# GuildOfWeavers/genSTARK

Measured on AMD Instinct MI355X. Metric: prove() ms + NTT GF(p) elements/sec, MiMC-128 2^20 steps, higher is better.
Workload: dtype u128; 1 GPU; MiMC-128 prove(), 2^20 steps, extensionFactor 16, exeQueryCount 48, friQueryCount 64, blake2s256; one independent proof per GPU; evaluation_domain=16777216, ntt_points_per_prove=17827072, ntt_transforms_per_prove=4, proof_bytes=371695

## Files before the change

### genstark_amd/_abi.py

```python
import ctypes as C
import os

_HERE = os.path.dirname(os.path.abspath(__file__))
HIP_LIB_PATH = os.path.join(_HERE, 'csrc', 'libgstark_hip.so')
MODULUS_128 = 2**128 - 9 * 2**32 + 1
MODULUS_64 = 2**64 - 21 * 2**30 + 1
MODULUS_32 = 2**32 - 3 * 2**25 + 1
MODULUS_17 = 96769
MODULUS_256 = 2**256 - 351 * 2**32 + 1
MODULUS_224 = 2**224 - 2**96 + 1
HIP_LIB_PATHS = {MODULUS_128: HIP_LIB_PATH, MODULUS_64: os.path.join(_HERE, 'csrc', 'libgstark_hip_q64.so'),
                 MODULUS_32: os.path.join(_HERE, 'csrc', 'libgstark_hip_q32.so'),
                 MODULUS_17: os.path.join(_HERE, 'csrc', 'libgstark_hip_q17.so'),
                 MODULUS_256: os.path.join(_HERE, 'csrc', 'libgstark_hip_p256.so'),
                 MODULUS_224: os.path.join(_HERE, 'csrc', 'libgstark_hip_p224.so')}
HIP_LIB_PATH_RUNTIME = os.path.join(_HERE, 'csrc', 'libgstark_hip_rt.so')

GS_OK = 0


class FriLayer(C.Structure):
    _fields_ = [('next', C.c_void_p), ('leaves', C.c_void_p), ('nodes', C.c_void_p), ('point_out', C.c_void_p), ('ticket', C.c_uint64)]

HASH_ALGS = {'sha256': 0, 'blake2s256': 1}
# ... 99 lines not shown
OPTIONAL_SYMBOLS = tuple(_OPTIONAL_SIGNATURES)

_HADES_SIGNATURES = {
    'gs_hades_create': (_int, [_vp, _u32, _u32, _u32, _u64, _bytes, _bytes, _pvp]),
    'gs_hades_destroy': (_int, [_vp, _vp]),
    'gs_hades_hash': (_int, [_vp, _vp, _vp, _u64, _u32, _u32, _vp]),
    'gs_hades_merkle': (_int, [_vp, _vp, _vp, _u64, _u32, _vp]),
    'gs_hades_merkle_paths': (_int, [_vp, _vp, _u64, _u32, C.POINTER(_u64), _u64, _vp]),
    'gs_hades_merkle_top': (_u32, []),
}
HADES_SYMBOLS = tuple(_HADES_SIGNATURES)

_RESCUE_SIGNATURES = {
    'gs_rescue_create': (_int, [_vp, _u32, _u32, _u64, _bytes, _bytes, _bytes, _pvp]),
    'gs_rescue_destroy': (_int, [_vp, _vp]),
    'gs_rescue_hash': (_int, [_vp, _vp, _vp, _u64, _u32, _u32, _u32, _u32, _vp]),
    'gs_rescue_merkle': (_int, [_vp, _vp, _vp, _u64, _vp]),
    'gs_rescue_spread_limit': (_u64, []),
}
RESCUE_SYMBOLS = tuple(_RESCUE_SIGNATURES)

_TREE_UPDATE_SIGNATURES = {
    'gs_hades_merkle_update': (_int, [_vp, _vp, _vp, _u64, _u32, C.POINTER(_u64), _vp, _u64, _vp, _vp]),
    'gs_rescue_merkle_update': (_int, [_vp, _vp, _vp, _u64, C.POINTER(_u64), _vp, _u64, _vp, _vp]),
}
TREE_UPDATE_SYMBOLS = tuple(_TREE_UPDATE_SIGNATURES)

_TREE_VERIFY_SIGNATURES = {
    'gs_hades_merkle_path_roots': (_int, [_vp, _vp, _vp, _u32, _u32, C.POINTER(_u64), _vp, _u64, _vp]),
    'gs_rescue_merkle_path_roots': (_int, [_vp, _vp, _vp, _u32, C.POINTER(_u64), _vp, _u64, _vp]),
}
TREE_VERIFY_SYMBOLS = tuple(_TREE_VERIFY_SIGNATURES)


class GstarkError(RuntimeError):
    pass


def load_library(path):
    if not os.path.exists(path):
        raise GstarkError(
            f'{path} not found: the HIP backend is not built (run `python -c "import __graft_entry__ as g; g.build()"`).'
            ' There is no CPU fallback.')
    lib = C.CDLL(path)
    for name, (res, args) in _SIGNATURES.items():
        fn = getattr(lib, name)
        fn.restype, fn.argtypes = res, args
    for name, (res, args) in (list(_OPTIONAL_SIGNATURES.items()) + list(_HADES_SIGNATURES.items()) + list(_RESCUE_SIGNATURES.items())
                              + list(_TREE_UPDATE_SIGNATURES.items()) + list(_TREE_VERIFY_SIGNATURES.items())):
        fn = getattr(lib, name, None)
        if fn is not None:
            fn.restype, fn.argtypes = res, args
    return lib


class Backend:

    def __init__(self, device=0, stream=None, lib_path=None, allow_test_double=False, modulus=None):
        if lib_path is None:
            lib_path = HIP_LIB_PATH if modulus is None else HIP_LIB_PATHS.get(modulus, HIP_LIB_PATH_RUNTIME)
        self.lib = load_library(lib_path)
        self.element_size = self.lib.gs_element_size()
        if modulus is not None:
            if modulus < 3 or modulus >> (8 * self.element_size):
                raise GstarkError(f'a modulus of {modulus.bit_length()} bits does not fit {lib_path}')
            rc = self.lib.gs_set_modulus(modulus.to_bytes(self.element_size, 'little'), self.element_size)
            if rc != GS_OK:
                raise GstarkError(f'{lib_path} does not compute modulo {modulus} (gs_set_modulus: {rc}'
                                  + (': the runtime-modulus library serves ONE modulus per process, and it has been given another' if rc == -3 else '') + ')')
        buf = C.create_string_buffer(self.element_size)
        self.lib.gs_field_modulus(C.cast(buf, C.c_void_p))
        self.modulus = int.from_bytes(buf.raw, 'little')
        if modulus is not None and self.modulus != modulus:
            raise GstarkError(f'{lib_path} is built for the field of {self.modulus} elements, not {modulus}')
        if not self.modulus:
            raise GstarkError(f'{lib_path} takes its modulus at run time: pass modulus=')
        self.name = self.lib.gs_backend_name().decode()
        if self.name != 'hip-gfx950' and not allow_test_double:
            raise GstarkError(f'refusing backend {self.name!r}: the product path runs on hip-gfx950 only')
        if self.lib.gs_abi_version() != 1:
            raise GstarkError('gstark ABI version mismatch')
        ctx = C.c_void_p()
# ... 86 lines not shown
```

### genstark_amd/csrc/air_mimc.hip

```cpp
#include "common.h"
#include "host_field.h"

__global__ void k_mimc_constraints(const fe *__restrict__ p, uint64_t nc, uint64_t shift, const fe *__restrict__ k, uint64_t klen,
                                   fe *__restrict__ out) {
    for (uint64_t j = blockIdx.x * (uint64_t)blockDim.x + threadIdx.x; j < nc; j += (uint64_t)gridDim.x * blockDim.x) {
        uint64_t jn = j + shift;
        if (jn >= nc) jn -= nc;
        fe x = p[j], nx = p[jn];
        fe x3 = fe_mul(fe_mul(x, x), x);
        out[j] = fe_sub(nx, fe_add(x3, k[j % klen]));
    }
}

#define GS_MIMC_COMP_MAX_PERIOD 32
#define GS_MIMC_COMP_MAX_ROOTS 4
struct MimcCompArgs {
    fe qz[GS_MIMC_COMP_MAX_PERIOD];
    fe bt[GS_MIMC_COMP_MAX_PERIOD];
    fe lt[GS_MIMC_COMP_MAX_PERIOD];
    fe ipoly[GS_MIMC_COMP_MAX_ROOTS];
    uint64_t root[GS_MIMC_COMP_MAX_ROOTS];
    fe x_last;
};
__global__ void k_mimc_composition(const fe *__restrict__ p, uint64_t n, uint64_t shift, const fe *__restrict__ k, uint64_t klen,
                                   const fe *__restrict__ tw_lo, const fe *__restrict__ tw_hi, int log_lo, int logn, const fe *__restrict__ u,
                                   MimcCompArgs a, uint32_t period, uint32_t nroots, int with_lc, fe *__restrict__ out) {
    __shared__ fe qz[GS_MIMC_COMP_MAX_PERIOD], bt[GS_MIMC_COMP_MAX_PERIOD], lt[GS_MIMC_COMP_MAX_PERIOD];
    if (threadIdx.x < period) { qz[threadIdx.x] = a.qz[threadIdx.x]; bt[threadIdx.x] = a.bt[threadIdx.x]; lt[threadIdx.x] = a.lt[threadIdx.x]; }
    __syncthreads();
    for (uint64_t i = blockIdx.x * (uint64_t)blockDim.x + threadIdx.x; i < n; i += (uint64_t)gridDim.x * blockDim.x) {
        fe x = tw_lo[i & ((1ull << log_lo) - 1)];
        if (logn > log_lo) x = fe_mul(x, tw_hi[i >> log_lo]);
        const fe pi = p[i], pn = p[(i + shift) & (n - 1)];
        const fe q = fe_sub(pn, fe_add(fe_mul(fe_mul(pi, pi), pi), k[i % klen]));
        const fe d = fe_mul(fe_mul(q, fe_sub(x, a.x_last)), qz[i & (period - 1)]);
        fe iv = a.ipoly[nroots - 1];
        for (int c = (int)nroots - 2; c >= 0; c--) iv = fe_add(fe_mul(iv, x), a.ipoly[c]);
        fe b = fe_mul(fe_sub(pi, iv), bt[i & (period - 1)]);
        for (uint32_t r = 0; r < nroots; r++) b = fe_mul(b, u[(i + n - a.root[r]) & (n - 1)]);
        fe r = fe_add(d, b);
        if (with_lc) r = fe_add(r, fe_mul(pi, lt[i & (period - 1)]));
        out[i] = r;
    }
}

#define GS_MIMC_CHUNK_BODY(STEP)                                                                                \
    for (uint64_t i = base; i < end; i++) {                                                                    \
        t[i] = hf_mimc_out(x);                                      \
        x = STEP(x, rc[ri]);                                   \
        if (++ri == nrc) ri = 0;                                                                               \
    }                                                                                                          \
    *ri_io = ri;                                                                                               \
    return x;
static hfe mimc_chunk_generic(hfe *t, hfe x, const hfe *rc, uint32_t nrc, uint32_t *ri_io, uint64_t base, uint64_t end) {
    uint32_t ri = *ri_io;
    GS_MIMC_CHUNK_BODY(hf_mimc_step_weak)
}
#if defined(__x86_64__) && !defined(__HIP_DEVICE_COMPILE__) && defined(GS_FIELD_128)
#define GS_MIMC_CHUNK_V3 1
__attribute__((target("arch=x86-64-v3,tune=znver5"))) static hfe mimc_chunk_v3(hfe *t, hfe x, const hfe *rc, uint32_t nrc, uint32_t *ri_io, uint64_t base,
                                                                               uint64_t end) {
    uint32_t ri = *ri_io;
    GS_MIMC_CHUNK_BODY(hf_cube_add_rows)
}
#endif
extern "C" {

int gs_mimc_trace(gs_ctx *c, const gs_elt *seed, const uint8_t *rc_host, uint32_t nrc, uint64_t steps, void *out) {
    if (!c || !seed || !rc_host || !out) return GS_ERR_ARG;
    if (!nrc || !steps) return gs_fail(c, GS_ERR_ARG, "mimc_trace: empty");
    std::vector<hfe> rc(nrc);
    for (uint32_t i = 0; i < nrc; i++) rc[i] = hf_load(rc_host + GS_ELT * i);
    int rcode = gs_trace_begin(c, steps * GS_ELT);
    if (rcode) return rcode;
    hfe *t = (hfe *)c->h_trace;
    hfe x = hf_load(seed);
    uint32_t ri = 0;
    const uint64_t CHUNK = 1ull << 16;
#ifdef GS_MIMC_CHUNK_V3
    static const bool v3 = __builtin_cpu_supports("avx2") && __builtin_cpu_supports("bmi2") && __builtin_cpu_supports("fma");
#else
    const bool v3 = false;
#endif
    for (uint64_t base = 0; base < steps; base += CHUNK) {
        const uint64_t end = base + CHUNK < steps ? base + CHUNK : steps;
#ifdef GS_MIMC_CHUNK_V3
        if (v3) x = mimc_chunk_v3(t, x, rc.data(), nrc, &ri, base, end);
        else
#endif
            x = mimc_chunk_generic(t, x, rc.data(), nrc, &ri, base, end);
        (void)v3;
        GS_HIP(c, hipMemcpyAsync((uint8_t *)out + base * GS_ELT, t + base, (end - base) * GS_ELT, hipMemcpyHostToDevice, c->stream));
    }
    return gs_trace_end(c);
}

int gs_mimc_constraints(gs_ctx *c, const void *p_comp, uint64_t nc, uint64_t shift, const void *k_table, uint64_t klen, void *out) {
    if (!c || !p_comp || !k_table || !out) return GS_ERR_ARG;
    if (!nc || !klen) return gs_fail(c, GS_ERR_ARG, "mimc_constraints: empty");
    hipLaunchKernelGGL(k_mimc_constraints, dim3(gs_grid(nc)), dim3(256), 0, c->stream, (const fe *)p_comp, nc, shift % nc,
                       (const fe *)k_table, klen, (fe *)out);
    GS_LAUNCH_CHECK(c);
    return GS_OK;
}

int gs_mimc_composition(gs_ctx *c, const void *p_eval, uint64_t n, uint64_t steps, const gs_elt *omega, const void *k_table, uint64_t klen,
                        const uint8_t *coeffs_host, uint64_t q_inc, uint64_t b_inc, const uint8_t *ipoly_host, const uint64_t *root_index_host,
                        uint32_t nroots, const uint8_t *lc_coeffs_host, void *out) {
    if (!c || !p_eval || !omega || !k_table || !coeffs_host || !ipoly_host || !root_index_host || !out) return GS_ERR_ARG;
    if (!gs_is_pow2(n) || !gs_is_pow2(steps) || steps > n || !klen) return gs_fail(c, GS_ERR_ARG, "mimc_composition: bad sizes");
    const uint64_t period = n / steps;
    if (period > GS_MIMC_COMP_MAX_PERIOD || nroots == 0 || nroots > GS_MIMC_COMP_MAX_ROOTS)
        return gs_fail(c, GS_ERR_UNSUPPORTED, "mimc_composition: n / steps <= %d and 1..%d assertions", GS_MIMC_COMP_MAX_PERIOD, GS_MIMC_COMP_MAX_ROOTS);
    if (q_inc % steps || b_inc % steps) return gs_fail(c, GS_ERR_ARG, "mimc_composition: degree increments must be multiples of the trace length");
    const fe w = fe_from_bytes(omega);
    const fe *lo, *hi, *u;
    int log_lo;
    int rc = gs_plan_pow_tables(c, w, n, &lo, &hi, &log_lo);
    if (!rc) rc = gs_plan_inverse_table(c, w, n, &u);
    if (rc) return rc;
    const fe d0 = fe_from_bytes(coeffs_host), d1 = fe_from_bytes(coeffs_host + GS_ELT), b0 = fe_from_bytes(coeffs_host + 2 * GS_ELT),
             b1 = fe_from_bytes(coeffs_host + 3 * GS_ELT);
    const fe l0 = lc_coeffs_host ? fe_from_bytes(lc_coeffs_host) : fe_zero(), l1 = lc_coeffs_host ? fe_from_bytes(lc_coeffs_host + GS_ELT) : fe_zero();
    MimcCompArgs a;
    uint64_t ksum = 0;
    for (uint32_t r = 0; r < GS_MIMC_COMP_MAX_ROOTS; r++) {
        a.root[r] = r < nroots ? root_index_host[r] & (n - 1) : 0;
        a.ipoly[r] = r < nroots ? fe_from_bytes(ipoly_host + GS_ELT * r) : fe_zero();
        if (r < nroots) ksum = (ksum + a.root[r]) & (n - 1);
    }
    const fe scale = gs_memo_pow(c, w, (n - ksum) & (n - 1));
    const std::vector<fe> &tab = gs_memo(c, gs_memo_key("mimc_comp").add(w).add(n).add(steps).add(q_inc).add(b_inc), [&](std::vector<fe> &t) {
        const fe g = fe_pow_u64(w, steps);
        const fe gq = fe_pow_u64(g, (q_inc / steps) % period), gb = fe_pow_u64(g, (b_inc / steps) % period);
        fe gj = fe_one(), gqj = fe_one(), gbj = fe_one();
        for (uint64_t j = 0; j < period; j++) {
            t.push_back(fe_inv(fe_sub(gj, fe_one())));
            t.push_back(gqj);
            t.push_back(gbj);
            gj = fe_mul(gj, g); gqj = fe_mul(gqj, gq); gbj = fe_mul(gbj, gb);
        }
        t.push_back(fe_pow_u64(w, (steps - 1) * period));
    });
    for (uint64_t j = 0; j < GS_MIMC_COMP_MAX_PERIOD; j++) {
        if (j < period) {
            a.qz[j] = fe_mul(fe_add(d0, fe_mul(d1, tab[3 * j + 1])), tab[3 * j]);
            a.bt[j] = fe_mul(fe_add(b0, fe_mul(b1, tab[3 * j + 2])), scale);
            a.lt[j] = fe_add(l0, fe_mul(l1, tab[3 * j + 2]));
        } else {
            a.qz[j] = a.bt[j] = a.lt[j] = fe_zero();
        }
    }
    a.x_last = tab[3 * period];
    gs_traffic(c, 2 * n * GS_ELT, n, "k_mimc_composition");
    hipLaunchKernelGGL(k_mimc_composition, dim3(gs_grid(n)), dim3(256), 0, c->stream, (const fe *)p_eval, n, period, (const fe *)k_table, klen, lo, hi,
                       log_lo, gs_log2(n), u, a, (uint32_t)period, nroots, lc_coeffs_host ? 1 : 0, (fe *)out);
    GS_LAUNCH_CHECK(c);
    return GS_OK;
}

}
```

### genstark_amd/csrc/common.h

```cpp
#pragma once
#include <hip/hip_runtime.h>
#include <stdint.h>
#include <stdio.h>
#include <stdarg.h>
#include <string.h>

#include <array>

#include <map>
#include <mutex>
#include <string>
#include <vector>

#include "../../include/gstark.h"
#if defined(GS_SMALL_Q)
#include "gf_small.h"
#elif defined(GS_WIDE_BITS)
#include "gf_wide.h"
#else
#include "gf128.h"
#define GS_FIELD_128 1
#endif

#if defined(GF_RUNTIME_MODULUS)
// ... 7 lines not shown

#define GS_ELT ((uint64_t)sizeof(fe))
#define GS_EW ((uint32_t)(sizeof(fe) / 16))
#ifndef GF_LIMBS
#define GF_LIMBS 4
GF_HD uint32_t fe_limb(const fe &a, int i) { return i == 0 ? a.w0 : (i == 1 ? a.w1 : (i == 2 ? a.w2 : a.w3)); }
GF_HD void fe_set_limb(fe &a, int i, uint32_t v) { if (i == 0) a.w0 = v; else if (i == 1) a.w1 = v; else if (i == 2) a.w2 = v; else a.w3 = v; }
#else
GF_HD uint32_t fe_limb(const fe &a, int i) { return a.w[i]; }
GF_HD void fe_set_limb(fe &a, int i, uint32_t v) { a.w[i] = v; }
#endif

struct NttPlan;

#define GS_HOST_TRACE_MAX_SEGMENTS 8

struct gs_ctx {
    int device = 0;
    hipStream_t stream = nullptr;
    bool own_stream = false;
    char err[512] = {0};
    std::mutex blocks_mutex;
    std::multimap<uint64_t, void *> free_blocks;
    std::map<void *, uint64_t> live_blocks;
    uint64_t cached_bytes = 0;
    std::map<std::string, NttPlan *> plans;
    void *h_stage = nullptr;
    void *h_stage_dev = nullptr;
    void *d_stage = nullptr;
    uint64_t stage_bytes = 0;
    void *fri_x = nullptr;
    void *fri_points = nullptr;
    std::map<std::string, std::vector<fe>> scalar_memo;
    uint64_t jit_launches = 0;
    bool traffic_on = false;
    std::map<std::string, std::array<uint64_t, 3>> traffic;
    uint64_t host_trace_segments = GS_HOST_TRACE_MAX_SEGMENTS;
    int air_jit = 2;
    struct DeferredCopy { void *dst; uint64_t first_word, bytes; };
    bool defer = false;
    std::vector<uint64_t> defer_addrs;
    std::vector<DeferredCopy> defer_copies;
    void *h_trace = nullptr;
    uint64_t trace_bytes = 0;
    hipEvent_t trace_done = nullptr;
    bool trace_pending = false;
    static constexpr uint32_t RB_SLOTS = 64, RB_SLOT_BYTES = 256;
    void *h_rb = nullptr, *h_rb_dev = nullptr;
    uint32_t rb_bytes[RB_SLOTS] = {};
    uint64_t rb_next = 0;
    void *h_fl = nullptr, *h_fl_dev = nullptr, *d_fl_count = nullptr;
    uint64_t fl_bytes = 0, fl_seq = 0;
    static constexpr uint64_t UP_HALF = 8ull << 20;
    void *h_up = nullptr;
    uint64_t up_off = 0;
    int up_half = 0;
    hipEvent_t up_done[2] = {};
    bool up_pending[2] = {false, false};
};

int gs_fail(gs_ctx *c, int code, const char *fmt, ...);

static inline void gs_traffic(gs_ctx *c, uint64_t bytes, uint64_t units, const char *fmt, ...) __attribute__((format(printf, 4, 5)));
static inline void gs_traffic(gs_ctx *c, uint64_t bytes, uint64_t units, const char *fmt, ...) {
    if (!c->traffic_on) return;
    char name[64];
// ... 74 lines not shown
```

### genstark_amd/csrc/gf128.h

```cpp
#pragma once
#include <stdint.h>

#if defined(__HIPCC__)
#define GF_HD __host__ __device__ __forceinline__
#else
#define GF_HD inline
#endif

struct alignas(16) fe {
    uint32_t w0, w1, w2, w3;
};

#define GF_P0 0x00000001u
#define GF_P1 0xFFFFFFF7u
#define GF_P2 0xFFFFFFFFu
#define GF_P3 0xFFFFFFFFu

GF_HD fe fe_make(uint32_t a, uint32_t b, uint32_t c, uint32_t d) { fe r; r.w0 = a; r.w1 = b; r.w2 = c; r.w3 = d; return r; }
GF_HD fe fe_zero() { return fe_make(0, 0, 0, 0); }
GF_HD fe fe_one() { return fe_make(1, 0, 0, 0); }
GF_HD bool fe_is_zero(const fe &a) { return (a.w0 | a.w1 | a.w2 | a.w3) == 0; }
GF_HD bool fe_eq(const fe &a, const fe &b) { return a.w0 == b.w0 && a.w1 == b.w1 && a.w2 == b.w2 && a.w3 == b.w3; }

GF_HD bool fe_ge_p(const fe &a) {
// ... 75 lines not shown
    o[2] = (uint32_t)t;
    t = (uint64_t)ai * b[3] + (t >> 32);
    o[3] = (uint32_t)t;
    o[4] = (uint32_t)(t >> 32);
}

GF_HD void fe_mul_wide(const fe &a, const fe &b, uint32_t r[8]) {
    const uint32_t bv[4] = {b.w0, b.w1, b.w2, b.w3};
    uint32_t r0[5], r1[5], r2[5], r3[5], c;
    fe_row_mul(a.w0, bv, r0);
    fe_row_mul(a.w1, bv, r1);
    fe_row_mul(a.w2, bv, r2);
    fe_row_mul(a.w3, bv, r3);
    r[0] = r0[0];
    r[1] = gf_addc(r0[1], r1[0], 0u, c);
    r[2] = gf_addc(r0[2], r1[1], c, c);
    r[3] = gf_addc(r0[3], r1[2], c, c);
    r[4] = gf_addc(r0[4], r1[3], c, c);
    r[5] = r1[4] + c;
    r[2] = gf_addc(r[2], r2[0], 0u, c);
    r[3] = gf_addc(r[3], r2[1], c, c);
    r[4] = gf_addc(r[4], r2[2], c, c);
    r[5] = gf_addc(r[5], r2[3], c, c);
    r[6] = r2[4] + c;
    r[3] = gf_addc(r[3], r3[0], 0u, c);
    r[4] = gf_addc(r[4], r3[1], c, c);
    r[5] = gf_addc(r[5], r3[2], c, c);
    r[6] = gf_addc(r[6], r3[3], c, c);
    r[7] = r3[4] + c;
}

GF_HD uint32_t gf_fsh(uint32_t hi, uint32_t lo, int s) { return (hi << s) | (lo >> (32 - s)); }

GF_HD fe fe_reduce_wide(const uint32_t r[8]) {
    uint32_t c, b;
    uint64_t m = (uint64_t)r[4] * 9u;
    uint32_t a0 = (uint32_t)m;
    m = (uint64_t)r[5] * 9u + (m >> 32);
    uint32_t a1 = (uint32_t)m;
    m = (uint64_t)r[6] * 9u + (m >> 32);
    uint32_t a2 = (uint32_t)m;
    m = (uint64_t)r[7] * 9u + (m >> 32);
    uint32_t a3 = (uint32_t)m, a4 = (uint32_t)(m >> 32);
    uint32_t u1 = gf_addc(r[1], a0, 0u, c);
    uint32_t u2 = gf_addc(r[2], a1, c, c);
    uint32_t u3 = gf_addc(r[3], a2, c, c);
    uint32_t u4 = gf_addc(a3, 0u, c, c);
    uint32_t u5 = a4 + c;
    uint32_t v0 = gf_subc(r[0], r[4], 0u, b);
    uint32_t v1 = gf_subc(u1, r[5], b, b);
    uint32_t v2 = gf_subc(u2, r[6], b, b);
    uint32_t v3 = gf_subc(u3, r[7], b, b);
    uint32_t t0 = gf_subc(u4, 0u, b, b);
    uint32_t t1 = u5 - b;
    uint32_t g0 = gf_addc(t0 << 3, t0, 0u, c);
    uint32_t g1 = gf_fsh(t1, t0, 3) + t1 + c;
    uint32_t e0 = gf_subc(0u, t0, 0u, b);
    uint32_t e1 = gf_subc(g0, t1, b, b);
    uint32_t e2 = g1 - b;
    fe w;
    uint32_t k;
    w.w0 = gf_addc(v0, e0, 0u, c);
    w.w1 = gf_addc(v1, e1, c, c);
    w.w2 = gf_addc(v2, e2, c, c);
    w.w3 = gf_addc(v3, 0u, c, k);
    fe t;
    t.w0 = gf_addc(w.w0, 0xFFFFFFFFu, 0u, c);
    t.w1 = gf_addc(w.w1, 8u, c, c);
    t.w2 = gf_addc(w.w2, 0u, c, c);
    t.w3 = gf_addc(w.w3, 0u, c, c);
    bool sel = (k | c) != 0;
    fe o;
    o.w0 = sel ? t.w0 : w.w0;
    o.w1 = sel ? t.w1 : w.w1;
    o.w2 = sel ? t.w2 : w.w2;
    o.w3 = sel ? t.w3 : w.w3;
    return o;
}

GF_HD fe fe_mul(const fe &a, const fe &b) {
    uint32_t r[8];
    fe_mul_wide(a, b, r);
    return fe_reduce_wide(r);
}
GF_HD fe fe_sqr(const fe &a) { return fe_mul(a, a); }

GF_HD fe fe_pow(fe b, const fe &e) {
    fe r = fe_one();
    const uint32_t ev[4] = {e.w0, e.w1, e.w2, e.w3};
    for (int i = 0; i < 4; i++) {
        uint32_t w = ev[i];
        for (int k = 0; k < 32; k++) {
            if (w & 1u) r = fe_mul(r, b);
            b = fe_sqr(b);
            w >>= 1;
        }
    }
    return r;
}
GF_HD fe fe_pow_u64(fe b, uint64_t e) {
    if (!e) return fe_one();
    fe r = b;
    bool have = false;
    for (;;) {
        if (e & 1u) { r = have ? fe_mul(r, b) : b; have = true; }
        e >>= 1;
        if (!e) break;
        b = fe_sqr(b);
    }
    return r;
// ... 35 lines not shown
```

### genstark_amd/csrc/prover.cc

```cpp
#include <dlfcn.h>
#include <stdarg.h>
#include <stdio.h>

#include <algorithm>
#include <map>
#include <chrono>
#include <deque>
#include <string>
#include <vector>

#include "../../include/gstark.h"
#include "../../include/gstark_prover.h"
#include "../../include/gstark_comm.h"
#include "../../include/gstark_boundary.h"
#if defined(GS_WIDE_BITS)
#include "gf_wide.h"
#endif
#include "host_field.h"
#include "host_poly.h"
#include "host_hash.h"

namespace {

#define GS_API_LIST(X)                                                                                                        \
    X(gs_alloc) X(gs_free) X(gs_upload) X(gs_download) X(gs_gather) X(gs_last_error) X(gs_power_series) X(gs_vec_add) X(gs_vec_mul) \
    X(gs_vec_sub_scalar) X(gs_vec_div) X(gs_combine_many) X(gs_combine_adjusted) X(gs_pluck) X(gs_transpose_vector) X(gs_sub_matrix_from_vectors)     \
    X(gs_eval_polys_at_roots) X(gs_interpolate_roots) X(gs_interpolate_quartic_domain) X(gs_eval_quartic_batch)                \
    X(gs_hash_merge_rows) X(gs_hash_digest_values) X(gs_merkle_build) X(gs_merkle_commit_rows) X(gs_merkle_prove_batch) X(gs_small_interpolate)          \
    X(gs_small_eval_poly) X(gs_pseudorandom_indexes) X(gs_mimc_trace) X(gs_mimc_constraints) X(gs_air_trace)                    \
    X(gs_air_trace_segments) X(gs_air_constraints) X(gs_air_constraints_strided) X(gs_composition_tail) X(gs_composition_tail_coset) X(gs_zero_poly_inverses) X(gs_div_by_domain_roots) X(gs_mimc_composition) X(gs_fri_fold) X(gs_fri_fold_seeded) X(gs_defer_begin) X(gs_defer_end) X(gs_readback_post) X(gs_readback_wait) X(gs_merkle_commit_rows_seed) X(gs_fri_fold_at) \
    X(gs_vec_mul_scalar) X(gs_copy) X(gs_gather_words) X(gs_transpose_records) X(gs_fri_fold_seeded_scaled) X(gs_fri_layers) X(gs_sync) X(gs_zero_poly_inverses_coset) X(gs_div_by_domain_roots_coset)
#define GS_API_OPTIONAL_LIST(X) X(gs_boundary_polys) X(gs_eval_polys_at_points)
struct Api {
#define X(name) decltype(&::name) name = nullptr;
    GS_API_LIST(X)
    GS_API_OPTIONAL_LIST(X)
#undef X
};
Api g_default_api;
bool g_bound = false;
thread_local const Api *g_api = &g_default_api;
#define A (*g_api)
struct UseApi {
    const Api *saved;
    explicit UseApi(const Api *a) : saved(g_api) { g_api = a; }
    ~UseApi() { g_api = saved; }
};

struct Fail {
    int code;
    std::string msg;
};
[[noreturn]] void fail(int code, const char *fmt, ...) {
    char buf[512];
    va_list ap;
    va_start(ap, fmt);
    vsnprintf(buf, sizeof buf, fmt, ap);
    va_end(ap);
    throw Fail{code, buf};
}

typedef hfe F;
const uint64_t ELEM = HF_ELT;
const uint64_t DIGEST = 32, MAX_ARRAY = 256;
const uint64_t WORD = 16, EW = ELEM / WORD;
// ... 900 lines not shown
    Plan plan = make_plan(job, T, E, omega, false);
    const uint64_t Nc = plan.Nc, combination_degree = plan.combination_degree, b_inc = plan.b_inc;
    const F comp_rou = hf_pow(omega, (hfe)(N / Nc)), exec_rou = hf_pow(omega, (hfe)E);
    const Coset domain{N, omega, 1, E, true};


    uint32_t assertions_on_r0 = 0;
    for (uint32_t i = 0; i < job.nassertions; i++) assertions_on_r0 += job.assertions[i].reg == 0;
    const bool fused = air.kind == 0 && E <= 32 && air.nconstraints == 1 && assertions_on_r0 == job.nassertions && job.nassertions <= 4;
    const bool tail = !fused && tail_fits(job, R + air.nsecret);
    const bool tail_makes_z = tail && domain.unit <= 32;
    uint32_t most_assertions = 0;
    for (auto &r : plan.regs) most_assertions = std::max(most_assertions, (uint32_t)r.steps.size());
    const uint32_t DEVICE_BOUNDARY_ABOVE = 128;
    const bool device_boundary = !fused && !tail && most_assertions > DEVICE_BOUNDARY_ABOVE && A.gs_boundary_polys && !g_host_boundary && plan.regs.size() <= 64 &&
                                 most_assertions <= T && T <= (1ull << 28);
    if (!device_boundary) plan.fill_xs();
    Buf zInverses;
    if (!fused && !tail_makes_z) zInverses = zero_poly_inverses(x, plan, domain);
    Buf psbPowers;
    const bool lc_folds = fused && R + air.nsecret == 1;
    if (b_inc > 0 && !lc_folds && !tail) psbPowers = coset_powers(x, domain, b_inc);

    Buf kN;
    uint64_t klen_n = 0;
    if (air.kind == 0) {
        klen_n = air.k_len * (N / Nc);
        Buf kPoly(x, air.k_len * ELEM);
        kN = Buf(x, klen_n * ELEM);
        x.check(counted_interpolate_roots(x.c, air.k_table, 1, enc(hf_pow(omega, (hfe)(N / air.k_len))), air.k_len, kPoly.p), "gs_interpolate_roots(K)");
        x.check(counted_eval_polys_at_roots(x.c, kPoly.p, 1, air.k_len, enc(hf_pow(omega, (hfe)(N / klen_n))), klen_n, kN.p), "gs_eval_polys_at_roots(K)");
    }

    clock.mark("context + trace-independent work issued");
    clock.readme(x, "Set up evaluation context");
    Buf trace(x, (uint64_t)R * T * ELEM);
    launch_trace(x, job, air.first_rows, air.segments, trace.p);
    check_assertion_ranges(job);
    std::vector<uint64_t> asserted_at;
    for (uint32_t i = 0; i < job.nassertions; i++) asserted_at.push_back((uint64_t)job.assertions[i].reg * T + job.assertions[i].step);

    clock.mark("execution trace (host recurrence)");
    clock.readme(x, "Generated execution trace");
    Buf pPolys(x, (uint64_t)R * T * ELEM), pEval(x, (uint64_t)R * N * ELEM);
    x.check(counted_interpolate_roots(x.c, trace.p, R, enc(exec_rou), T, pPolys.p), "gs_interpolate_roots(trace)");
    clock.readme(x, "Computed execution trace polynomials P(x)");
    x.check(counted_eval_polys_at_roots(x.c, pPolys.p, R, T, enc(omega), N, pEval.p), "gs_eval_polys_at_roots(P)");
    clock.readme(x, "Low-degree extended P(x) polynomials over evaluation domain");
    std::vector<const void *> pRows(R);
    for (uint32_t r = 0; r < R; r++) pRows[r] = pEval.at((uint64_t)r * N * ELEM);
    std::vector<const void *> eVectors(pRows);
    for (uint32_t i = 0; i < air.nsecret; i++) eVectors.push_back(air.secret_traces[i]);
    const uint32_t V = (uint32_t)eVectors.size();

    Tree eTree = commit_rows(x, alg, eVectors.data(), V, N, false);

    clock.mark("P(x), extension, evaluation tree issued");
    clock.readme(x, "Serialized evaluations of P(x) and S(x) polynomials + Built evaluation merkle tree (one fused call)");
    const uint32_t dcount = plan.dcount, bcoef = plan.bcoef;
    std::vector<F> coefficients;
    auto read_evaluation_root = [&] {
        Bytes got(asserted_at.size() * ELEM);
        const uint64_t one = 1;
        DeferWindow win(x);
        x.check(A.gs_gather(x.c, trace.p, ELEM, asserted_at.data(), asserted_at.size(), got.data()), "gs_gather(asserted cells)");
        x.check(A.gs_gather(x.c, eTree.nodes.p, DIGEST, &one, 1, eTree.root.data()), "gs_gather(root)");
        win.end();
        check_asserted_cells(job, [&](uint32_t i) { return got.data() + i * ELEM; });
        trace.release();
        coefficients = plan.coefficients(eTree.root, V);
    };

    Buf cEval(x, N * ELEM);
    bool lc_fused = false;
    if (fused) {
        const Plan::Boundary bd = plan.boundary(E, true);
        read_evaluation_root();
        const bool q_adjusted = plan.groups[0].first < combination_degree;
        Bytes co(4 * ELEM, 0);
        store_elem(coefficients[0], co.data());
        if (q_adjusted) store_elem(coefficients[1], co.data() + ELEM);
        store_elem(coefficients[dcount], co.data() + 2 * ELEM);
        if (b_inc > 0) store_elem(coefficients[dcount + 1], co.data() + 3 * ELEM);
        lc_fused = lc_folds;
        Bytes lc = lc_folds ? pack(coefficients, dcount + bcoef, plan.lccount(V)) : Bytes();
        lc.resize(2 * ELEM, 0);
        x.check(A.gs_mimc_composition(x.c, pRows[0], N, T, enc(omega), kN.p, klen_n, co.data(), q_adjusted ? combination_degree - plan.groups[0].first : 0, b_inc,
                                      bd.interpolants.data(), bd.at.data(), bd.per_row[0], lc_folds ? lc.data() : nullptr, cEval.p), "gs_mimc_composition");
    } else {
        const bool direct = air.kind == 0;
        const Coset qDomain = direct ? domain : Coset{Nc, comp_rou, 1, Nc / T, true};
        const uint64_t Nq = qDomain.n;
        Buf q(x, (uint64_t)air.nconstraints * Nq * ELEM);
        if (direct) {
            x.check(A.gs_mimc_constraints(x.c, pRows[0], N, N / T, kN.p, klen_n, q.p), "gs_mimc_constraints");
        } else {
            x.check(A.gs_air_constraints_strided(x.c, air.e_code, air.e_ninstr, air.consts, air.nconsts, air.vm_regs, R, air.nconstraints, pEval.p, N, N / Nc,
                                                 Nc, Nc / T, air.static_tables, air.static_lens, air.nstatic, q.p), "gs_air_constraints_strided");
        }
        std::vector<const void *> qa;
        for (uint32_t i = 0; i < air.nconstraints; i++) qa.push_back(q.at((uint64_t)i * Nq * ELEM));
        read_evaluation_root();
        Buf qe(x, N * ELEM), qc;
        if (!direct) qc = Buf(x, Nc * ELEM);
        merge_q(x, plan, coefficients, qa, Nq, [&](uint64_t e) { return coset_powers(x, qDomain, e); }, direct ? qe.p : qc.p);
        if (!direct) {
            Buf qcPoly(x, Nc * ELEM);
            x.check(counted_interpolate_roots(x.c, qc.p, 1, enc(comp_rou), Nc, qcPoly.p), "gs_interpolate_roots(Q)");
            x.check(counted_eval_polys_at_roots(x.c, qcPoly.p, 1, Nc, enc(omega), N, qe.p), "gs_eval_polys_at_roots(Q)");
        }
        std::vector<const void *> pv;
        for (auto &r : plan.regs) pv.push_back(pRows[r.reg]);
        if (tail) {
            composition_tail(x, plan, domain, coefficients, qe.p, tail_makes_z ? nullptr : zInverses.p, pv, eVectors, cEval.p);
            lc_fused = true;
        } else {
            member_sequence(x, plan, domain, device_boundary, coefficients, qe, zInverses, pv, psbPowers, cEval.p);
        }
    }
    zInverses.release();

// ... 92 lines not shown
```

Before: 1.667 billion elements/s.

## Precompute cached X/U/IU tables for MiMC composition and fuse the reduction dot product

Adds a prepare step, issued before trace generation, that builds three device tables. They hold x - x_last, the product of shifted inverse values for the assertion roots, and that product multiplied by the boundary interpolant. X and U are cached in the context by domain and root keys; IU is rebuilt whenever the interpolant changes. The composition kernel then reads these tables instead of evaluating powers, gathering inverse entries and running the interpolant Horner loop per point. It also combines the three final products with a single lazy 128-bit reduction (new fe_reduce_wide9). The cost is three extra N-element buffers, a large amount of memory at this domain size, and more memory traffic in the composition kernel in exchange for less arithmetic.

```diff
diff --git a/genstark_amd/_abi.py b/genstark_amd/_abi.py
--- a/genstark_amd/_abi.py
+++ b/genstark_amd/_abi.py
@@ -155,6 +155,13 @@
 }
 TREE_VERIFY_SYMBOLS = tuple(_TREE_VERIFY_SIGNATURES)
 
+_MIMC_SIGNATURES = {
+    'gs_mimc_composition_prepare': (_int, [_vp, _u64, _u64, _bytes, C.POINTER(_u64), _u32, _bytes]),
+    'gs_mimc_composition_tables': _SIGNATURES['gs_mimc_composition'],
+    'gs_mimc_composition_tables_max_n': (_u64, [_u64]),
+}
+MIMC_SYMBOLS = tuple(_MIMC_SIGNATURES)
+
 
 class GstarkError(RuntimeError):
     pass
@@ -170,7 +177,7 @@
         fn = getattr(lib, name)
         fn.restype, fn.argtypes = res, args
     for name, (res, args) in (list(_OPTIONAL_SIGNATURES.items()) + list(_HADES_SIGNATURES.items()) + list(_RESCUE_SIGNATURES.items())
-                              + list(_TREE_UPDATE_SIGNATURES.items()) + list(_TREE_VERIFY_SIGNATURES.items())):
+                              + list(_TREE_UPDATE_SIGNATURES.items()) + list(_TREE_VERIFY_SIGNATURES.items()) + list(_MIMC_SIGNATURES.items())):
         fn = getattr(lib, name, None)
         if fn is not None:
             fn.restype, fn.argtypes = res, args
diff --git a/genstark_amd/csrc/air_mimc.hip b/genstark_amd/csrc/air_mimc.hip
--- a/genstark_amd/csrc/air_mimc.hip
+++ b/genstark_amd/csrc/air_mimc.hip
@@ -1,5 +1,8 @@
 #include "common.h"
 #include "host_field.h"
+#include "../../include/gstark_mimc.h"
+
+#include <atomic>
 
 __global__ void k_mimc_constraints(const fe *__restrict__ p, uint64_t nc, uint64_t shift, const fe *__restrict__ k, uint64_t klen,
                                    fe *__restrict__ out) {
@@ -44,6 +47,65 @@
     }
 }
 
+__global__ void k_mimc_table_x(const fe *__restrict__ tw_lo, const fe *__restrict__ tw_hi, int log_lo, int logn, uint64_t n, fe x_last,
+                               fe *__restrict__ X) {
+    for (uint64_t i = blockIdx.x * (uint64_t)blockDim.x + threadIdx.x; i < n; i += (uint64_t)gridDim.x * blockDim.x) {
+        fe x = tw_lo[i & ((1ull << log_lo) - 1)];
+        if (logn > log_lo) x = fe_mul(x, tw_hi[i >> log_lo]);
+        X[i] = fe_sub(x, x_last);
+    }
+}
+struct MimcRoots {
+    uint64_t root[GS_MIMC_COMP_MAX_ROOTS];
+    fe ipoly[GS_MIMC_COMP_MAX_ROOTS];
+};
+__global__ void k_mimc_table_u(const fe *__restrict__ u, uint64_t n, MimcRoots a, uint32_t nroots, fe *__restrict__ U) {
+    for (uint64_t i = blockIdx.x * (uint64_t)blockDim.x + threadIdx.x; i < n; i += (uint64_t)gridDim.x * blockDim.x) {
+        fe v = u[(i + n - a.root[0]) & (n - 1)];
+        for (uint32_t r = 1; r < nroots; r++) v = fe_mul(v, u[(i + n - a.root[r]) & (n - 1)]);
+        U[i] = v;
+    }
+}
+__global__ void k_mimc_table_iu(const fe *__restrict__ X, const fe *__restrict__ U, uint64_t n, MimcRoots a, uint32_t nroots, fe x_last,
+                                fe *__restrict__ IU) {
+    for (uint64_t i = blockIdx.x * (uint64_t)blockDim.x + threadIdx.x; i < n; i += (uint64_t)gridDim.x * blockDim.x) {
+        const fe x = fe_add(X[i], x_last);
+        fe iv = a.ipoly[nroots - 1];
+        for (int c = (int)nroots - 2; c >= 0; c--) iv = fe_add(fe_mul(iv, x), a.ipoly[c]);
+        IU[i] = fe_mul(iv, U[i]);
+    }
+}
+__device__ __forceinline__ fe mimc_dot(const fe &a0, const fe &b0, const fe &a1, const fe &b1, const fe &a2, const fe &b2, bool three) {
+#ifdef GS_FIELD_128
+    uint32_t s[8], t[8], top = 0;
+    fe_mul_wide(a0, b0, s);
+    fe_mul_wide(a1, b1, t);
+    fe_wide_add(s, t, top);
+    if (three) {
+        fe_mul_wide(a2, b2, t);
+        fe_wide_add(s, t, top);
+    }
+    return fe_reduce_wide9(s, top);
+#else
+    const fe r = fe_add(fe_mul(a0, b0), fe_mul(a1, b1));
+    return three ? fe_add(r, fe_mul(a2, b2)) : r;
+#endif
+}
+__global__ void k_mimc_composition_tables(const fe *__restrict__ p, uint64_t n, uint64_t shift, const fe *__restrict__ k, uint64_t klen,
+                                          const fe *__restrict__ X, const fe *__restrict__ U, const fe *__restrict__ IU, MimcCompArgs a,
+                                          uint32_t period, int with_lc, fe *__restrict__ out) {
+    __shared__ fe qz[GS_MIMC_COMP_MAX_PERIOD], bt[GS_MIMC_COMP_MAX_PERIOD], lt[GS_MIMC_COMP_MAX_PERIOD];
+    if (threadIdx.x < period) { qz[threadIdx.x] = a.qz[threadIdx.x]; bt[threadIdx.x] = a.bt[threadIdx.x]; lt[threadIdx.x] = a.lt[threadIdx.x]; }
+    __syncthreads();
+    const bool kpow2 = !(klen & (klen - 1));
+    for (uint64_t i = blockIdx.x * (uint64_t)blockDim.x + threadIdx.x; i < n; i += (uint64_t)gridDim.x * blockDim.x) {
+        const fe pi = p[i], pn = p[(i + shift) & (n - 1)];
+        const fe q = fe_sub(pn, fe_add(fe_mul(fe_mul(pi, pi), pi), k[kpow2 ? i & (klen - 1) : i % klen]));
+        const uint32_t j = (uint32_t)i & (period - 1);
+        out[i] = mimc_dot(fe_mul(q, X[i]), qz[j], fe_sub(fe_mul(pi, U[i]), IU[i]), bt[j], pi, lt[j], with_lc != 0);
+    }
+}
+
 #define GS_MIMC_CHUNK_BODY(STEP)                                                                                \
     for (uint64_t i = base; i < end; i++) {                                                                    \
         t[i] = hf_mimc_out(x);                                      \
@@ -64,6 +126,81 @@
     GS_MIMC_CHUNK_BODY(hf_cube_add_rows)
 }
 #endif
+
+static int mimc_comp_check(gs_ctx *c, uint64_t n, uint64_t steps, uint64_t klen, uint64_t q_inc, uint64_t b_inc, uint32_t nroots) {
+    if (!gs_is_pow2(n) || !gs_is_pow2(steps) || steps > n || !klen) return gs_fail(c, GS_ERR_ARG, "mimc_composition: bad sizes");
+    if (n / steps > GS_MIMC_COMP_MAX_PERIOD || nroots == 0 || nroots > GS_MIMC_COMP_MAX_ROOTS)
+        return gs_fail(c, GS_ERR_UNSUPPORTED, "mimc_composition: n / steps <= %d and 1..%d assertions", GS_MIMC_COMP_MAX_PERIOD, GS_MIMC_COMP_MAX_ROOTS);
+    if (q_inc % steps || b_inc % steps) return gs_fail(c, GS_ERR_ARG, "mimc_composition: degree increments must be multiples of the trace length");
+    return GS_OK;
+}
+static fe mimc_x_last(gs_ctx *c, const fe &w, uint64_t n, uint64_t steps) { return gs_memo_pow(c, w, (steps - 1) * (n / steps)); }
+static void mimc_comp_args(gs_ctx *c, const fe &w, uint64_t n, uint64_t steps, const uint8_t *coeffs_host, uint64_t q_inc, uint64_t b_inc,
+                           const uint8_t *ipoly_host, const uint64_t *root_index_host, uint32_t nroots, const uint8_t *lc_coeffs_host, MimcCompArgs &a) {
+    const uint64_t period = n / steps;
+    const fe d0 = fe_from_bytes(coeffs_host), d1 = fe_from_bytes(coeffs_host + GS_ELT), b0 = fe_from_bytes(coeffs_host + 2 * GS_ELT),
+             b1 = fe_from_bytes(coeffs_host + 3 * GS_ELT);
+    const fe l0 = lc_coeffs_host ? fe_from_bytes(lc_coeffs_host) : fe_zero(), l1 = lc_coeffs_host ? fe_from_bytes(lc_coeffs_host + GS_ELT) : fe_zero();
+    uint64_t ksum = 0;
+    for (uint32_t r = 0; r < GS_MIMC_COMP_MAX_ROOTS; r++) {
+        a.root[r] = r < nroots ? root_index_host[r] & (n - 1) : 0;
+        a.ipoly[r] = r < nroots ? fe_from_bytes(ipoly_host + GS_ELT * r) : fe_zero();
+        if (r < nroots) ksum = (ksum + a.root[r]) & (n - 1);
+    }
+    const fe scale = gs_memo_pow(c, w, (n - ksum) & (n - 1));
+    const std::vector<fe> &tab = gs_memo(c, gs_memo_key("mimc_comp").add(w).add(n).add(steps).add(q_inc).add(b_inc), [&](std::vector<fe> &t) {
+        const fe g = fe_pow_u64(w, steps);
+        const fe gq = fe_pow_u64(g, (q_inc / steps) % period), gb = fe_pow_u64(g, (b_inc / steps) % period);
+        fe gj = fe_one(), gqj = fe_one(), gbj = fe_one();
+        for (uint64_t j = 0; j < period; j++) {
+            t.push_back(fe_inv(fe_sub(gj, fe_one())));
+            t.push_back(gqj);
+            t.push_back(gbj);
+            gj = fe_mul(gj, g); gqj = fe_mul(gqj, gq); gbj = fe_mul(gbj, gb);
+        }
+        t.push_back(fe_pow_u64(w, (steps - 1) * period));
+    });
+    for (uint64_t j = 0; j < GS_MIMC_COMP_MAX_PERIOD; j++) {
+        if (j < period) {
+            a.qz[j] = fe_mul(fe_add(d0, fe_mul(d1, tab[3 * j + 1])), tab[3 * j]);
+            a.bt[j] = fe_mul(fe_add(b0, fe_mul(b1, tab[3 * j + 2])), scale);
+            a.lt[j] = fe_add(l0, fe_mul(l1, tab[3 * j + 2]));
+        } else {
+            a.qz[j] = a.bt[j] = a.lt[j] = fe_zero();
+        }
+    }
+    a.x_last = tab[3 * period];
+}
+
+static MimcRoots mimc_roots(uint64_t n, const uint64_t *root_index_host, uint32_t nroots, const uint8_t *ipoly_host) {
+    MimcRoots a;
+    for (uint32_t r = 0; r < GS_MIMC_COMP_MAX_ROOTS; r++) {
+        a.root[r] = r < nroots ? root_index_host[r] & (n - 1) : 0;
+        a.ipoly[r] = r < nroots ? fe_from_bytes(ipoly_host + GS_ELT * r) : fe_zero();
+    }
+    return a;
+}
+static std::string mimc_x_key(const fe &w, uint64_t n, uint64_t steps) { return gs_memo_key("X").add(w).add(n).add(steps).k; }
+static std::string mimc_u_key(const std::string &x_key, const uint64_t *root, uint32_t nroots) {
+    gs_memo_key k("U");
+    k.add(x_key.data(), x_key.size()).add((uint64_t)nroots);
+    for (uint32_t r = 0; r < nroots; r++) k.add(root[r]);
+    return k.k;
+}
+static std::string mimc_iu_key(const std::string &u_key, const fe *ipoly, uint32_t nroots) {
+    gs_memo_key k("IU");
+    k.add(u_key.data(), u_key.size());
+    for (uint32_t r = 0; r < nroots; r++) k.add(ipoly[r]);
+    return k.k;
+}
+static void mimc_tables_drop(gs_ctx *c) {
+    gs_ctx::MimcTables &t = c->mimc_tables;
+    gs_free(c, t.X); gs_free(c, t.U); gs_free(c, t.IU);
+    t = gs_ctx::MimcTables();
+}
+#define GS_MIMC_TABLES_MAX_N (1ull << 26)
+static std::atomic<uint64_t> g_mimc_tables_max_n{GS_MIMC_TABLES_MAX_N};
+
 extern "C" {
 
 int gs_mimc_trace(gs_ctx *c, const gs_elt *seed, const uint8_t *rc_host, uint32_t nrc, uint64_t steps, void *out) {
@@ -108,50 +245,17 @@
                         const uint8_t *coeffs_host, uint64_t q_inc, uint64_t b_inc, const uint8_t *ipoly_host, const uint64_t *root_index_host,
                         uint32_t nroots, const uint8_t *lc_coeffs_host, void *out) {
     if (!c || !p_eval || !omega || !k_table || !coeffs_host || !ipoly_host || !root_index_host || !out) return GS_ERR_ARG;
-    if (!gs_is_pow2(n) || !gs_is_pow2(steps) || steps > n || !klen) return gs_fail(c, GS_ERR_ARG, "mimc_composition: bad sizes");
+    int rc = mimc_comp_check(c, n, steps, klen, q_inc, b_inc, nroots);
+    if (rc) return rc;
+    const fe w = fe_from_bytes(omega);
     const uint64_t period = n / steps;
-    if (period > GS_MIMC_COMP_MAX_PERIOD || nroots == 0 || nroots > GS_MIMC_COMP_MAX_ROOTS)
-        return gs_fail(c, GS_ERR_UNSUPPORTED, "mimc_composition: n / steps <= %d and 1..%d assertions", GS_MIMC_COMP_MAX_PERIOD, GS_MIMC_COMP_MAX_ROOTS);
-    if (q_inc % steps || b_inc % steps) return gs_fail(c, GS_ERR_ARG, "mimc_composition: degree increments must be multiples of the trace length");
-    const fe w = fe_from_bytes(omega);
     const fe *lo, *hi, *u;
     int log_lo;
-    int rc = gs_plan_pow_tables(c, w, n, &lo, &hi, &log_lo);
+    rc = gs_plan_pow_tables(c, w, n, &lo, &hi, &log_lo);
     if (!rc) rc = gs_plan_inverse_table(c, w, n, &u);
     if (rc) return rc;
-    const fe d0 = fe_from_bytes(coeffs_host), d1 = fe_from_bytes(coeffs_host + GS_ELT), b0 = fe_from_bytes(coeffs_host + 2 * GS_ELT),
-             b1 = fe_from_bytes(coeffs_host + 3 * GS_ELT);
-    const fe l0 = lc_coeffs_host ? fe_from_bytes(lc_coeffs_host) : fe_zero(), l1 = lc_coeffs_host ? fe_from_bytes(lc_coeffs_host + GS_ELT) : fe_zero();
     MimcCompArgs a;
-    uint64_t ksum = 0;
-    for (uint32_t r = 0; r < GS_MIMC_COMP_MAX_ROOTS; r++) {
-        a.root[r] = r < nroots ? root_index_host[r] & (n - 1) : 0;
-        a.ipoly[r] = r < nroots ? fe_from_bytes(ipoly_host + GS_ELT * r) : fe_zero();
-        if (r < nroots) ksum = (ksum + a.root[r]) & (n - 1);
-    }
-    const fe scale = gs_memo_pow(c, w, (n - ksum) & (n - 1));
-    const std::vector<fe> &tab = gs_memo(c, gs_memo_key("mimc_comp").add(w).add(n).add(steps).add(q_inc).add(b_inc), [&](std::vector<fe> &t) {
-        const fe g = fe_pow_u64(w, steps);
-        const fe gq = fe_pow_u64(g, (q_inc / steps) % period), gb = fe_pow_u64(g, (b_inc / steps) % period);
-        fe gj = fe_one(), gqj = fe_one(), gbj = fe_one();
-        for (uint64_t j = 0; j < period; j++) {
-            t.push_back(fe_inv(fe_sub(gj, fe_one())));
-            t.push_back(gqj);
-            t.push_back(gbj);
-            gj = fe_mul(gj, g); gqj = fe_mul(gqj, gq); gbj = fe_mul(gbj, gb);
-        }
-        t.push_back(fe_pow_u64(w, (steps - 1) * period));
-    });
-    for (uint64_t j = 0; j < GS_MIMC_COMP_MAX_PERIOD; j++) {
-        if (j < period) {
-            a.qz[j] = fe_mul(fe_add(d0, fe_mul(d1, tab[3 * j + 1])), tab[3 * j]);
-            a.bt[j] = fe_mul(fe_add(b0, fe_mul(b1, tab[3 * j + 2])), scale);
-            a.lt[j] = fe_add(l0, fe_mul(l1, tab[3 * j + 2]));
-        } else {
-            a.qz[j] = a.bt[j] = a.lt[j] = fe_zero();
-        }
-    }
-    a.x_last = tab[3 * period];
+    mimc_comp_args(c, w, n, steps, coeffs_host, q_inc, b_inc, ipoly_host, root_index_host, nroots, lc_coeffs_host, a);
     gs_traffic(c, 2 * n * GS_ELT, n, "k_mimc_composition");
     hipLaunchKernelGGL(k_mimc_composition, dim3(gs_grid(n)), dim3(256), 0, c->stream, (const fe *)p_eval, n, period, (const fe *)k_table, klen, lo, hi,
                        log_lo, gs_log2(n), u, a, (uint32_t)period, nroots, lc_coeffs_host ? 1 : 0, (fe *)out);
@@ -159,4 +263,79 @@
     return GS_OK;
 }
 
-}
+uint64_t gs_mimc_composition_tables_max_n(uint64_t max_n) {
+    return g_mimc_tables_max_n.exchange(max_n && max_n < GS_MIMC_TABLES_MAX_N ? max_n : GS_MIMC_TABLES_MAX_N);
+}
+
+int gs_mimc_composition_prepare(gs_ctx *c, uint64_t n, uint64_t steps, const gs_elt *omega, const uint64_t *root_index_host, uint32_t nroots,
+                                const uint8_t *ipoly_host) {
+    if (!c || !omega || !root_index_host || !ipoly_host) return GS_ERR_ARG;
+    int rc = mimc_comp_check(c, n, steps, 1, 0, 0, nroots);
+    if (rc) return rc;
+    gs_ctx::MimcTables &t = c->mimc_tables;
+    t.iu_key.clear();
+    if (n > g_mimc_tables_max_n.load()) { mimc_tables_drop(c); return GS_OK; }
+    const fe w = fe_from_bytes(omega);
+    const fe *lo, *hi, *u;
+    int log_lo;
+    rc = gs_plan_pow_tables(c, w, n, &lo, &hi, &log_lo);
+    if (!rc) rc = gs_plan_inverse_table(c, w, n, &u);
+    if (rc) return rc;
+    if (t.n != n) {
+        mimc_tables_drop(c);
+        void *q[3] = {nullptr, nullptr, nullptr};
+        for (int i = 0; i < 3 && !rc; i++) rc = gs_alloc(c, n * GS_ELT, &q[i]);
+        if (rc) {
+            for (int i = 0; i < 3; i++) gs_free(c, q[i]);
+            return GS_OK;
+        }
+        t.X = (fe *)q[0]; t.U = (fe *)q[1]; t.IU = (fe *)q[2];
+        t.n = n;
+    }
+    const MimcRoots a = mimc_roots(n, root_index_host, nroots, ipoly_host);
+    const fe x_last = mimc_x_last(c, w, n, steps);
+    const dim3 grid(gs_grid(n)), block(256);
+    const std::string x_key = mimc_x_key(w, n, steps), u_key = mimc_u_key(x_key, a.root, nroots);
+    const bool make_x = t.x_key != x_key, make_u = t.u_key != u_key;
+    if (make_x) {
+        t.x_key.clear();
+        gs_traffic(c, n * GS_ELT, n, "k_mimc_table_x");
+        hipLaunchKernelGGL(k_mimc_table_x, grid, block, 0, c->stream, lo, hi, log_lo, gs_log2(n), n, x_last, t.X);
+    }
+    if (make_u) {
+        t.u_key.clear();
+        gs_traffic(c, 2 * n * GS_ELT, n * (nroots - 1), "k_mimc_table_u");
+        hipLaunchKernelGGL(k_mimc_table_u, grid, block, 0, c->stream, u, n, a, nroots, t.U);
+    }
+    gs_traffic(c, 3 * n * GS_ELT, n * nroots, "k_mimc_table_iu");
+    hipLaunchKernelGGL(k_mimc_table_iu, grid, block, 0, c->stream, t.X, t.U, n, a, nroots, x_last, t.IU);
+    GS_LAUNCH_CHECK(c);
+    t.x_key = x_key;
+    t.u_key = u_key;
+    t.iu_key = mimc_iu_key(u_key, a.ipoly, nroots);
+    return GS_OK;
+}
+
+int gs_mimc_composition_tables(gs_ctx *c, const void *p_eval, uint64_t n, uint64_t steps, const gs_elt *omega, const void *k_table, uint64_t klen,
+                               const uint8_t *coeffs_host, uint64_t q_inc, uint64_t b_inc, const uint8_t *ipoly_host, const uint64_t *root_index_host,
+                               uint32_t nroots, const uint8_t *lc_coeffs_host, void *out) {
+    if (!c || !p_eval || !omega || !k_table || !coeffs_host || !ipoly_host || !root_index_host || !out) return GS_ERR_ARG;
+    int rc = mimc_comp_check(c, n, steps, klen, q_inc, b_inc, nroots);
+    if (rc) return rc;
+    const fe w = fe_from_bytes(omega);
+    const gs_ctx::MimcTables &t = c->mimc_tables;
+    const MimcRoots ra = mimc_roots(n, root_index_host, nroots, ipoly_host);
+    if (t.iu_key.empty() || t.n != n || t.iu_key != mimc_iu_key(mimc_u_key(mimc_x_key(w, n, steps), ra.root, nroots), ra.ipoly, nroots))
+        return gs_mimc_composition(c, p_eval, n, steps, omega, k_table, klen, coeffs_host, q_inc, b_inc, ipoly_host, root_index_host, nroots,
+                                   lc_coeffs_host, out);
+    MimcCompArgs a;
+    mimc_comp_args(c, w, n, steps, coeffs_host, q_inc, b_inc, ipoly_host, root_index_host, nroots, lc_coeffs_host, a);
+    const uint64_t period = n / steps;
+    gs_traffic(c, 5 * n * GS_ELT, n, "k_mimc_composition_tables");
+    hipLaunchKernelGGL(k_mimc_composition_tables, dim3(gs_grid(n)), dim3(256), 0, c->stream, (const fe *)p_eval, n, period, (const fe *)k_table, klen,
+                       t.X, t.U, t.IU, a, (uint32_t)period, lc_coeffs_host ? 1 : 0, (fe *)out);
+    GS_LAUNCH_CHECK(c);
+    return GS_OK;
+}
+
+}
diff --git a/genstark_amd/csrc/common.h b/genstark_amd/csrc/common.h
--- a/genstark_amd/csrc/common.h
+++ b/genstark_amd/csrc/common.h
@@ -63,6 +63,11 @@
     void *fri_x = nullptr;
     void *fri_points = nullptr;
     std::map<std::string, std::vector<fe>> scalar_memo;
+    struct MimcTables {
+        fe *X = nullptr, *U = nullptr, *IU = nullptr;
+        uint64_t n = 0;
+        std::string x_key, u_key, iu_key;
+    } mimc_tables;
     uint64_t jit_launches = 0;
     bool traffic_on = false;
     std::map<std::string, std::array<uint64_t, 3>> traffic;
diff --git a/genstark_amd/csrc/gf128.h b/genstark_amd/csrc/gf128.h
--- a/genstark_amd/csrc/gf128.h
+++ b/genstark_amd/csrc/gf128.h
@@ -131,7 +131,7 @@
 
 GF_HD uint32_t gf_fsh(uint32_t hi, uint32_t lo, int s) { return (hi << s) | (lo >> (32 - s)); }
 
-GF_HD fe fe_reduce_wide(const uint32_t r[8]) {
+GF_HD fe fe_reduce_wide9(const uint32_t r[8], uint32_t r8) {
     uint32_t c, b;
     uint64_t m = (uint64_t)r[4] * 9u;
     uint32_t a0 = (uint32_t)m;
@@ -140,7 +140,9 @@
     m = (uint64_t)r[6] * 9u + (m >> 32);
     uint32_t a2 = (uint32_t)m;
     m = (uint64_t)r[7] * 9u + (m >> 32);
-    uint32_t a3 = (uint32_t)m, a4 = (uint32_t)(m >> 32);
+    uint32_t a3 = (uint32_t)m;
+    m = (uint64_t)r8 * 9u + (m >> 32);
+    uint32_t a4 = (uint32_t)m;
     uint32_t u1 = gf_addc(r[1], a0, 0u, c);
     uint32_t u2 = gf_addc(r[2], a1, c, c);
     uint32_t u3 = gf_addc(r[3], a2, c, c);
@@ -150,7 +152,7 @@
     uint32_t v1 = gf_subc(u1, r[5], b, b);
     uint32_t v2 = gf_subc(u2, r[6], b, b);
     uint32_t v3 = gf_subc(u3, r[7], b, b);
-    uint32_t t0 = gf_subc(u4, 0u, b, b);
+    uint32_t t0 = gf_subc(u4, r8, b, b);
     uint32_t t1 = u5 - b;
     uint32_t g0 = gf_addc(t0 << 3, t0, 0u, c);
     uint32_t g1 = gf_fsh(t1, t0, 3) + t1 + c;
@@ -175,6 +177,14 @@
     o.w2 = sel ? t.w2 : w.w2;
     o.w3 = sel ? t.w3 : w.w3;
     return o;
+}
+GF_HD fe fe_reduce_wide(const uint32_t r[8]) { return fe_reduce_wide9(r, 0u); }
+GF_HD void fe_wide_add(uint32_t x[8], const uint32_t y[8], uint32_t &top) {
+    uint32_t c;
+    x[0] = gf_addc(x[0], y[0], 0u, c);
+#pragma unroll
+    for (int i = 1; i < 8; i++) x[i] = gf_addc(x[i], y[i], c, c);
+    top += c;
 }
 
 GF_HD fe fe_mul(const fe &a, const fe &b) {
diff --git a/genstark_amd/csrc/prover.cc b/genstark_amd/csrc/prover.cc
--- a/genstark_amd/csrc/prover.cc
+++ b/genstark_amd/csrc/prover.cc
@@ -13,6 +13,7 @@
 #include "../../include/gstark_prover.h"
 #include "../../include/gstark_comm.h"
 #include "../../include/gstark_boundary.h"
+#include "../../include/gstark_mimc.h"
 #if defined(GS_WIDE_BITS)
 #include "gf_wide.h"
 #endif
@@ -30,7 +31,7 @@
     X(gs_small_eval_poly) X(gs_pseudorandom_indexes) X(gs_mimc_trace) X(gs_mimc_constraints) X(gs_air_trace)                    \
     X(gs_air_trace_segments) X(gs_air_constraints) X(gs_air_constraints_strided) X(gs_composition_tail) X(gs_composition_tail_coset) X(gs_zero_poly_inverses) X(gs_div_by_domain_roots) X(gs_mimc_composition) X(gs_fri_fold) X(gs_fri_fold_seeded) X(gs_defer_begin) X(gs_defer_end) X(gs_readback_post) X(gs_readback_wait) X(gs_merkle_commit_rows_seed) X(gs_fri_fold_at) \
     X(gs_vec_mul_scalar) X(gs_copy) X(gs_gather_words) X(gs_transpose_records) X(gs_fri_fold_seeded_scaled) X(gs_fri_layers) X(gs_sync) X(gs_zero_poly_inverses_coset) X(gs_div_by_domain_roots_coset)
-#define GS_API_OPTIONAL_LIST(X) X(gs_boundary_polys) X(gs_eval_polys_at_points)
+#define GS_API_OPTIONAL_LIST(X) X(gs_boundary_polys) X(gs_eval_polys_at_points) X(gs_mimc_composition_prepare) X(gs_mimc_composition_tables)
 struct Api {
 #define X(name) decltype(&::name) name = nullptr;
     GS_API_LIST(X)
@@ -997,6 +998,21 @@
         x.check(counted_eval_polys_at_roots(x.c, kPoly.p, 1, air.k_len, enc(hf_pow(omega, (hfe)(N / klen_n))), klen_n, kN.p), "gs_eval_polys_at_roots(K)");
     }
 
+    Plan::Boundary fused_bd;
+    bool comp_tables = false;
+    if (fused && A.gs_mimc_composition_prepare && A.gs_mimc_composition_tables) {
+        const std::vector<uint64_t> &at = plan.regs[0].steps;
+        bool sound = true;
+        for (size_t i = 0; i < at.size(); i++) {
+            if (at[i] >= T) sound = false;
+            for (size_t k = 0; k < i; k++) if (at[k] == at[i]) sound = false;
+        }
+        if (sound) {
+            fused_bd = plan.boundary(E, true);
+            comp_tables = A.gs_mimc_composition_prepare(x.c, N, T, enc(omega), fused_bd.at.data(), fused_bd.per_row[0], fused_bd.interpolants.data()) == GS_OK;
+        }
+    }
+
     clock.mark("context + trace-independent work issued");
     clock.readme(x, "Set up evaluation context");
     Buf trace(x, (uint64_t)R * T * ELEM);
@@ -1039,7 +1055,7 @@
     Buf cEval(x, N * ELEM);
     bool lc_fused = false;
     if (fused) {
-        const Plan::Boundary bd = plan.boundary(E, true);
+        const Plan::Boundary bd = comp_tables ? std::move(fused_bd) : plan.boundary(E, true);
         read_evaluation_root();
         const bool q_adjusted = plan.groups[0].first < combination_degree;
         Bytes co(4 * ELEM, 0);
@@ -1050,8 +1066,10 @@
         lc_fused = lc_folds;
         Bytes lc = lc_folds ? pack(coefficients, dcount + bcoef, plan.lccount(V)) : Bytes();
         lc.resize(2 * ELEM, 0);
-        x.check(A.gs_mimc_composition(x.c, pRows[0], N, T, enc(omega), kN.p, klen_n, co.data(), q_adjusted ? combination_degree - plan.groups[0].first : 0, b_inc,
-                                      bd.interpolants.data(), bd.at.data(), bd.per_row[0], lc_folds ? lc.data() : nullptr, cEval.p), "gs_mimc_composition");
+        const auto composition = comp_tables ? A.gs_mimc_composition_tables : A.gs_mimc_composition;
+        x.check(composition(x.c, pRows[0], N, T, enc(omega), kN.p, klen_n, co.data(), q_adjusted ? combination_degree - plan.groups[0].first : 0, b_inc,
+                            bd.interpolants.data(), bd.at.data(), bd.per_row[0], lc_folds ? lc.data() : nullptr, cEval.p),
+                comp_tables ? "gs_mimc_composition_tables" : "gs_mimc_composition");
     } else {
         const bool direct = air.kind == 0;
         const Coset qDomain = direct ? domain : Coset{Nc, comp_rou, 1, Nc / T, true};
diff --git a/include/gstark_mimc.h b/include/gstark_mimc.h
--- /dev/null
+++ b/include/gstark_mimc.h
@@ -0,0 +1,23 @@
+#ifndef GSTARK_MIMC_H
+#define GSTARK_MIMC_H
+
+#include "gstark.h"
+
+#ifdef __cplusplus
+extern "C" {
+#endif
+
+int gs_mimc_composition_prepare(gs_ctx *ctx, uint64_t n, uint64_t steps, const gs_elt *omega, const uint64_t *root_index_host, uint32_t nroots,
+                                const uint8_t *ipoly_host);
+
+int gs_mimc_composition_tables(gs_ctx *ctx, const void *p_eval, uint64_t n, uint64_t steps, const gs_elt *omega, const void *k_table,
+                               uint64_t klen, const uint8_t *coeffs_host, uint64_t q_inc, uint64_t b_inc, const uint8_t *ipoly_host,
+                               const uint64_t *root_index_host, uint32_t nroots, const uint8_t *lc_coeffs_host, void *out);
+
+uint64_t gs_mimc_composition_tables_max_n(uint64_t max_n);
+
+#ifdef __cplusplus
+}
+#endif
+
+#endif
```

Measured after the change: 1.697 billion elements/s (median of 6 runs). 1.8% higher.
